# MVPandey/DTS

Measured on AMD Instinct MI355X. Metric: scored_trajectories_per_sec, higher is better.
Workload: dtype bf16

## Files before the change

dts_amd/models/llama.py:

```python

from __future__ import annotations

import math
from typing import Optional

import torch
import torch.nn as nn
import torch.nn.functional as F

from dts_amd import ops
from dts_amd.models.config import ModelSpec
from dts_amd.ops.torch_ref import build_rope_cache
from dts_amd.parallel.tp import (
    ColumnParallelLinear,
    RowParallelLinear,
    TPContext,
    _init_weight,
)
from dts_amd.serving.batch import ForwardBatch


class LlamaAttention(nn.Module):
    def __init__(self, spec: ModelSpec, tp: TPContext, dtype):
        super().__init__()
        self.tp = tp
        assert spec.num_heads % tp.size == 0
        assert spec.num_kv_heads % tp.size == 0 or tp.size % spec.num_kv_heads == 0
        self.num_heads = spec.num_heads // tp.size
        self.num_kv_heads = max(1, spec.num_kv_heads // tp.size)
        self.head_dim = spec.head_dim
        self.scale = 1.0 / math.sqrt(spec.head_dim)
        q_out = self.num_heads * self.head_dim * tp.size
        kv_out = self.num_kv_heads * self.head_dim * tp.size
        self.qkv_proj = ColumnParallelLinear(
            spec.hidden_size, q_out + 2 * kv_out, tp, dtype=dtype
        )
        self.o_proj = RowParallelLinear(
            self.num_heads * self.head_dim * tp.size, spec.hidden_size, tp, dtype=dtype
        )
        self.q_size = self.num_heads * self.head_dim
        self.kv_size = self.num_kv_heads * self.head_dim

    def forward(
        self,
        hidden: torch.Tensor,
        batch: ForwardBatch,
        kv_layer: tuple,
        rope: tuple,
    ) -> torch.Tensor:
        T = hidden.shape[0]
        qkv = self.qkv_proj(hidden)
        q, k, v = qkv.split([self.q_size, self.kv_size, self.kv_size], dim=-1)
        q = q.view(T, self.num_heads, self.head_dim)
        k = k.view(T, self.num_kv_heads, self.head_dim)
        v = v.view(T, self.num_kv_heads, self.head_dim)

        k_cache, v_cache = kv_layer
        cos, sin = rope
        q, k = ops.rope_kv_append(
            q, k, v, batch.positions, cos, sin, k_cache, v_cache, batch.slot_mapping
        )

        out = torch.empty(q.shape, dtype=q.dtype, device=q.device)
        np_tok = batch.num_prefill_tokens
        if batch.num_prefill_seqs:
            ops.attn_prefill_paged(
                q[:np_tok],
                batch.cu_q,
                batch.positions[:np_tok],
                k_cache,
                v_cache,
                batch.prefill_block_tables,
                batch.prefill_kv_lens,
                self.scale,
                out=out[:np_tok],
            )
        if batch.num_decode_seqs:
            ops.attn_decode_paged(
                q[np_tok:],
                k_cache,
                v_cache,
                batch.decode_block_tables,
                batch.decode_kv_lens,
                self.scale,
                out=out[np_tok:],
            )
        return self.o_proj(out.reshape(T, -1))


class LlamaMLP(nn.Module):
    def __init__(self, spec: ModelSpec, tp: TPContext, dtype):
        super().__init__()
        self.gate_up_proj = ColumnParallelLinear(
            spec.hidden_size, 2 * spec.intermediate_size, tp, dtype=dtype
        )
        self.down_proj = RowParallelLinear(
            spec.intermediate_size, spec.hidden_size, tp, dtype=dtype
        )
        self.inter_per_rank = spec.intermediate_size // tp.size

    def forward(self, x: torch.Tensor) -> torch.Tensor:
        gu = self.gate_up_proj(x)
        return self.down_proj(ops.silu_mul(gu))


class LlamaLayer(nn.Module):
    def __init__(self, spec: ModelSpec, tp: TPContext, dtype):
        super().__init__()
        self.input_norm_w = nn.Parameter(
            torch.ones(spec.hidden_size, dtype=dtype), requires_grad=False
        )
        self.post_norm_w = nn.Parameter(
            torch.ones(spec.hidden_size, dtype=dtype), requires_grad=False
        )
        self.attn = LlamaAttention(spec, tp, dtype)
        self.mlp = LlamaMLP(spec, tp, dtype)
        self.eps = spec.rms_eps

    def forward(self, hidden, residual, batch, kv_layer, rope):
        if residual is None:
            residual = hidden
            hidden = ops.rmsnorm(hidden, self.input_norm_w, self.eps)
        else:
            hidden, residual = ops.fused_add_rmsnorm(
                hidden, residual, self.input_norm_w, self.eps
            )
        hidden = self.attn(hidden, batch, kv_layer, rope)
        hidden, residual = ops.fused_add_rmsnorm(
            hidden, residual, self.post_norm_w, self.eps
        )
        hidden = self.mlp(hidden)
        return hidden, residual


class LlamaModel(nn.Module):
    arch = "llama"

    def __init__(
        self,
        spec: ModelSpec,
        tp: Optional[TPContext] = None,
        dtype: torch.dtype = torch.bfloat16,
        device: str = "cpu",
    ):
        super().__init__()
        tp = tp or TPContext.single()
        self.spec = spec
        self.tp = tp
        self.dtype = dtype
        self.num_kv_heads_local = max(1, spec.num_kv_heads // tp.size)
        self.embed = nn.Parameter(
            torch.empty(spec.vocab_size, spec.hidden_size, dtype=dtype),
            requires_grad=False,
        )
        self.layers = nn.ModuleList(
            [LlamaLayer(spec, tp, dtype) for _ in range(spec.num_layers)]
        )
        self.final_norm_w = nn.Parameter(
            torch.ones(spec.hidden_size, dtype=dtype), requires_grad=False
        )
        self.lm_head = ColumnParallelLinear(
            spec.hidden_size, spec.vocab_size, tp, dtype=dtype, gather_output=True
        )
        cos, sin = build_rope_cache(
            spec.head_dim, spec.max_position, spec.rope_theta, dtype=torch.float32
        )
        self.register_buffer("rope_cos", cos, persistent=False)
        self.register_buffer("rope_sin", sin, persistent=False)
        self.to(device)

    def random_init(self, seed: int = 0) -> None:
        dev = self.embed.device
        g = torch.Generator(device=dev).manual_seed(seed)
        spec = self.spec
        with torch.no_grad():
            self.embed.copy_(
                torch.randn(
                    spec.vocab_size, spec.hidden_size, generator=g, device=dev
                )
                .mul_(0.02)
                .to(self.dtype)
            )
            for layer in self.layers:
                for lin in (
                    layer.attn.qkv_proj,
                    layer.attn.o_proj,
                    layer.mlp.gate_up_proj,
                    layer.mlp.down_proj,
                ):
                    lin.weight.copy_(
                        _init_weight(
                            *lin.weight.shape,
                            dtype=self.dtype,
                            generator=g,
                            device=dev,
                        )
                    )
            self.lm_head.weight.copy_(
                _init_weight(
                    *self.lm_head.weight.shape,
                    dtype=self.dtype,
                    generator=g,
                    device=dev,
                )
            )

    def forward(self, batch: ForwardBatch, kv_pool) -> torch.Tensor:
        hidden = self.embed[batch.token_ids]
        residual = None
        rope = (self.rope_cos, self.rope_sin)
        for i, layer in enumerate(self.layers):
            hidden, residual = layer(hidden, residual, batch, kv_pool.layer(i), rope)
        hidden, _ = ops.fused_add_rmsnorm(
            hidden, residual, self.final_norm_w, self.spec.rms_eps
        )
        if batch.sample_indices is not None:
            hidden = hidden[batch.sample_indices]
        return self.lm_head(hidden).float()
```

dts_amd/ops/__init__.py:

```python

from __future__ import annotations

import os

import torch

from dts_amd.ops import torch_ref
from dts_amd.utils.logging import logger

_hip = None
_hip_load_error: Exception | None = None


def _try_load_hip():
    global _hip, _hip_load_error
    if _hip is not None or _hip_load_error is not None:
        return _hip
    try:
        from dts_amd.ops import _hip_ext_loader

        _hip = _hip_ext_loader.load()
        logger.info("HIP extension loaded: %s", _hip.__name__)
    except Exception as e:
        _hip_load_error = e
    return _hip


def hip_available() -> bool:
    return _try_load_hip() is not None


def _require_hip():
    ext = _try_load_hip()
    if ext is None:
        if os.environ.get("DTS_ALLOW_TORCH_FALLBACK") == "1":
            return None
        raise RuntimeError(
            "dts_amd HIP extension not available on a GPU device "
            f"(load error: {_hip_load_error}); refusing silent eager fallback. "
            "Build with `python -m dts_amd.ops.build` or set "
            "DTS_ALLOW_TORCH_FALLBACK=1 for debugging."
        )
    return ext


def _on_gpu(t: torch.Tensor) -> bool:
    return t.is_cuda



def rmsnorm(x, weight, eps=1e-5):
    if _on_gpu(x):
        ext = _require_hip()
        if ext is not None:
            out = torch.empty_like(x)
            ext.rmsnorm(out, x, weight, eps)
            return out
    return torch_ref.rmsnorm(x, weight, eps)


def fused_add_rmsnorm(x, residual, weight, eps=1e-5):
    if _on_gpu(x):
        ext = _require_hip()
        if ext is not None:
            ext.fused_add_rmsnorm(x, residual, weight, eps)
            return x, residual
    return torch_ref.fused_add_rmsnorm(x, residual, weight, eps)


def layernorm(x, weight, bias, eps=1e-5):
    if _on_gpu(x):
        ext = _require_hip()
        if ext is not None:
            out = torch.empty_like(x)
            ext.layernorm(out, x, weight, bias, eps)
            return out
    return torch_ref.layernorm(x, weight, bias, eps)


def rope_kv_append(q, k, v, positions, cos, sin, k_cache, v_cache, slot_mapping):
    if _on_gpu(q):
        ext = _require_hip()
        if ext is not None:
            ext.rope_kv_append(q, k, v, positions, cos, sin, k_cache, v_cache, slot_mapping)
            return q, k
    q, k = torch_ref.rope_apply(q, k, positions, cos, sin)
    torch_ref.kv_append(k, v, k_cache, v_cache, slot_mapping)
    return q, k


def kv_append(k, v, k_cache, v_cache, slot_mapping):
    if _on_gpu(k):
        ext = _require_hip()
        if ext is not None:
            ext.kv_append(k, v, k_cache, v_cache, slot_mapping)
            return
    torch_ref.kv_append(k, v, k_cache, v_cache, slot_mapping)


def attn_prefill_paged(
    q, cu_q, q_positions, k_cache, v_cache, block_tables, kv_lens, scale=None,
    out=None,
):
    if _on_gpu(q):
        ext = _require_hip()
        if ext is not None:
            import math

            if out is None or not out.is_contiguous():
                out = torch.empty(q.shape, dtype=q.dtype, device=q.device)
            ext.attn_prefill_paged(
                out, q, cu_q, q_positions, k_cache, v_cache, block_tables, kv_lens,
                scale if scale is not None else 1.0 / math.sqrt(q.shape[-1]),
            )
            return out
    ref = torch_ref.attn_prefill_paged(
        q, cu_q, q_positions, k_cache, v_cache, block_tables, kv_lens, scale
    )
    if out is not None:
        out.copy_(ref)
        return out
    return ref


def attn_decode_paged(q, k_cache, v_cache, block_tables, kv_lens, scale=None, out=None):
    if _on_gpu(q):
        ext = _require_hip()
        if ext is not None:
            import math

            if out is None or not out.is_contiguous():
                out = torch.empty(q.shape, dtype=q.dtype, device=q.device)
            ext.attn_decode_paged(
                out, q, k_cache, v_cache, block_tables, kv_lens,
                scale if scale is not None else 1.0 / math.sqrt(q.shape[-1]),
            )
            return out
    ref = torch_ref.attn_decode_paged(q, k_cache, v_cache, block_tables, kv_lens, scale)
    if out is not None:
        out.copy_(ref)
        return out
    return ref


def silu_mul(gate_up):
    if gate_up.shape[0] == 0:
        return gate_up[:, : gate_up.shape[1] // 2]
    if _on_gpu(gate_up):
        ext = _require_hip()
        if ext is not None:
            T = gate_up.shape[0]
            out = torch.empty(
                (T, gate_up.shape[1] // 2), dtype=gate_up.dtype, device=gate_up.device
            )
            ext.silu_mul(out, gate_up)
            return out
    return torch_ref.silu_mul(gate_up)


def gelu(x):
    return torch_ref.gelu(x)


_sampler_ws: dict = {}


def _sampler_workspace(S: int, device):
    key = (str(device), S)
    ws = _sampler_ws.get(key)
    if ws is None:
        ws = (
            torch.zeros(S, dtype=torch.int64, device=device),
            torch.zeros(S, 1024, dtype=torch.float32, device=device),
            torch.zeros(S, 16, dtype=torch.float32, device=device),
            torch.zeros(S, dtype=torch.float32, device=device),
        )
        _sampler_ws[key] = ws
    return ws


def top_p_sample(logits, temperatures, top_ps, generators=None, seeds=None, out=None):
    if _on_gpu(logits):
        ext = _require_hip()
        if ext is not None and seeds is not None:
            S, V = logits.shape
            if out is None:
                out = torch.empty(S, dtype=torch.long, device=logits.device)
            if V >= 4096 and S <= 32 and os.environ.get("DTS_SAMPLER_V1") != "1":
                ws = _sampler_workspace(S, logits.device)
                ext.top_p_sample_v2(
                    out, logits, temperatures, top_ps, seeds, *ws
                )
            else:
                ext.top_p_sample(out, logits, temperatures, top_ps, seeds)
            return out
    return torch_ref.top_p_sample(logits, temperatures, top_ps, generators)


def derive_seeds(out, bases, positions):
    if _on_gpu(out):
        ext = _require_hip()
        if ext is not None:
            ext.derive_seeds(out, bases, positions)
            return out
    out.copy_(torch_ref.derive_seeds(bases, positions))
    return out


mix_seed = torch_ref.mix_seed


def moe_grouped_linear(x, w, counts, offsets):
    if _on_gpu(x):
        ext = _require_hip()
        if ext is not None:
            out = torch.empty(
                (x.shape[0], w.shape[1]), dtype=x.dtype, device=x.device
            )
            ext.moe_grouped_linear(out, x, w, counts, offsets)
            return out
    return torch_ref.moe_grouped_linear(x, w, counts, offsets)


def linear_bf16(x: torch.Tensor, weight: torch.Tensor) -> torch.Tensor:
    M = x.shape[0] if x.dim() == 2 else 0
    if (
        x.is_cuda
        and x.dtype == torch.bfloat16
        and x.dim() == 2
        and x.shape[1] % 512 == 0
        and weight.stride(1) == 1
        and 1 <= M <= 16
    ):
        ext = _require_hip()
        if ext is not None:
            out = torch.empty(
                (M, weight.shape[0]), dtype=x.dtype, device=x.device
            )
            big = weight.shape[0] * weight.shape[1] * 2 > (96 << 20)
            if M <= 2 and big and x.shape[1] <= 8192:
                ext.gemv_bf16(out, x, weight)
            else:
                ext.gemm_skinny_bf16(out, x, weight)
            return out
    return torch.nn.functional.linear(x, weight)
```

dts_amd/ops/hip/bindings.cpp:

```cpp
#include <torch/extension.h>

void rmsnorm(torch::Tensor out, torch::Tensor x, torch::Tensor w, double eps);
void fused_add_rmsnorm(torch::Tensor x, torch::Tensor residual,
                       torch::Tensor w, double eps);
void silu_mul(torch::Tensor out, torch::Tensor in);
void layernorm(torch::Tensor out, torch::Tensor x, torch::Tensor w,
               torch::Tensor b, double eps);
void rope_kv_append(torch::Tensor q, torch::Tensor k, torch::Tensor v,
                    torch::Tensor positions, torch::Tensor cos_t,
                    torch::Tensor sin_t, torch::Tensor k_cache,
                    torch::Tensor v_cache, torch::Tensor slots);
void kv_append(torch::Tensor k, torch::Tensor v, torch::Tensor k_cache,
               torch::Tensor v_cache, torch::Tensor slots);
void attn_decode_paged(torch::Tensor out, torch::Tensor q,
                       torch::Tensor kcache, torch::Tensor vcache,
                       torch::Tensor block_tables, torch::Tensor kv_lens,
                       double scale);
void attn_prefill_paged(torch::Tensor out, torch::Tensor q, torch::Tensor cu_q,
                        torch::Tensor q_pos, torch::Tensor kcache,
                        torch::Tensor vcache, torch::Tensor block_tables,
                        torch::Tensor kv_lens, double scale, int64_t swz);
void top_p_sample(torch::Tensor out, torch::Tensor logits, torch::Tensor temps,
                  torch::Tensor top_ps, torch::Tensor seeds);
void derive_seeds(torch::Tensor out, torch::Tensor bases,
                  torch::Tensor positions);
void top_p_sample_v2(torch::Tensor out, torch::Tensor logits,
                     torch::Tensor temps, torch::Tensor top_ps,
                     torch::Tensor seeds, torch::Tensor ws_max,
                     torch::Tensor ws_bins, torch::Tensor ws_slice,
                     torch::Tensor ws_tau);
void gemv_bf16(torch::Tensor out, torch::Tensor x, torch::Tensor w);
void gemm_skinny_bf16(torch::Tensor out, torch::Tensor x, torch::Tensor w);
void moe_grouped_linear(torch::Tensor out, torch::Tensor x, torch::Tensor w,
                        torch::Tensor counts, torch::Tensor offsets);

PYBIND11_MODULE(TORCH_EXTENSION_NAME, m) {
  m.def("rmsnorm", &rmsnorm, "RMSNorm (bf16, CDNA4)");
  m.def("fused_add_rmsnorm", &fused_add_rmsnorm,
        "fused residual add + RMSNorm (in-place, bf16)");
  m.def("silu_mul", &silu_mul, "SwiGLU activation (bf16)");
  m.def("layernorm", &layernorm, "LayerNorm (bf16, GPT-2 path)");
  m.def("rope_kv_append", &rope_kv_append,
        "fused rotate-half RoPE + paged KV append (bf16)");
  m.def("kv_append", &kv_append, "paged KV append without RoPE (bf16)");
  m.def("attn_decode_paged", &attn_decode_paged,
        "paged GQA decode attention (bf16, wave-per-kv-head)");
  m.def("attn_prefill_paged", &attn_prefill_paged,
        "paged causal prefill attention (bf16, MFMA)", py::arg("out"),
        py::arg("q"), py::arg("cu_q"), py::arg("q_pos"), py::arg("kcache"),
        py::arg("vcache"), py::arg("block_tables"), py::arg("kv_lens"),
        py::arg("scale"), py::arg("swz") = -1);
  m.def("top_p_sample", &top_p_sample,
        "fused temperature softmax + top-p sampling (sort-free)");
  m.def("derive_seeds", &derive_seeds,
        "stateless (seed, position) mix for chained decode");
  m.def("top_p_sample_v2", &top_p_sample_v2,
        "gridded top-p sampler (vocab sliced across workgroups)");
  m.def("gemv_bf16", &gemv_bf16,
        "skinny-batch (M<=8) bf16 weight-streaming GEMV");
  m.def("gemm_skinny_bf16", &gemm_skinny_bf16,
        "skinny-M (M<=16) bf16 MFMA weight-streaming GEMM");
  m.def("moe_grouped_linear", &moe_grouped_linear,
        "grouped per-expert skinny GEMM (capture-safe MoE decode)");
}
```

dts_amd/ops/hip/common.h:

```cpp
#pragma once

#include <hip/hip_runtime.h>
#include <hip/hip_bf16.h>
#include <hip/hip_fp16.h>

#define WAVE 64
#define DEV __device__ __forceinline__

typedef __attribute__((ext_vector_type(4))) short short4v;
typedef __attribute__((ext_vector_type(8))) short short8v;
typedef __attribute__((ext_vector_type(4))) float float4v;

DEV float bf2f(short u) {
  union { float f; unsigned int i; } c;
  c.i = ((unsigned int)(unsigned short)u) << 16;
  return c.f;
}

DEV short f2bf(float f) {
  union { float f; unsigned int i; } c;
  c.f = f;
  unsigned int lsb = (c.i >> 16) & 1;
  c.i += 0x7fff + lsb;
  return (short)(c.i >> 16);
}

DEV float wave_sum(float v) {
#pragma unroll
  for (int off = 32; off > 0; off >>= 1) v += __shfl_xor(v, off, 64);
  return v;
}

DEV float wave_max(float v) {
#pragma unroll
  for (int off = 32; off > 0; off >>= 1) v = fmaxf(v, __shfl_xor(v, off, 64));
  return v;
}

#define HIP_CHECK_LAST()                                                      \
  do {                                                                        \
    hipError_t e = hipGetLastError();                                         \
    if (e != hipSuccess) {                                                    \
      TORCH_CHECK(false, "HIP kernel launch failed: ", hipGetErrorString(e)); \
    }                                                                         \
  } while (0)
```

dts_amd/ops/hip/elementwise.hip:

```cpp

#include "common.h"
#include <torch/extension.h>
#include <c10/hip/HIPStream.h>


template <int BLOCK>
__global__ void rmsnorm_kernel(short* __restrict__ out,
                               const short* __restrict__ x,
                               const short* __restrict__ w, float eps, int T,
                               int H) {
  __shared__ float red[BLOCK / WAVE];
  for (int row = blockIdx.x; row < T; row += gridDim.x) {
    const short* xr = x + (long)row * H;
    short* yr = out + (long)row * H;
    float ss = 0.f;
    for (int i = threadIdx.x * 8; i < H; i += BLOCK * 8) {
      short8v v = *(const short8v*)(xr + i);
#pragma unroll
      for (int j = 0; j < 8; ++j) {
        float f = bf2f(v[j]);
        ss += f * f;
      }
    }
    ss = wave_sum(ss);
    if ((threadIdx.x & (WAVE - 1)) == 0) red[threadIdx.x / WAVE] = ss;
    __syncthreads();
    float tot = 0.f;
#pragma unroll
    for (int i = 0; i < BLOCK / WAVE; ++i) tot += red[i];
    float inv = rsqrtf(tot / H + eps);
    for (int i = threadIdx.x * 8; i < H; i += BLOCK * 8) {
      short8v v = *(const short8v*)(xr + i);
      short8v wv = *(const short8v*)(w + i);
      short8v o;
#pragma unroll
      for (int j = 0; j < 8; ++j) o[j] = f2bf(bf2f(v[j]) * inv * bf2f(wv[j]));
      *(short8v*)(yr + i) = o;
    }
    __syncthreads();
  }
}


template <int BLOCK>
__global__ void fused_add_rmsnorm_kernel(short* __restrict__ x,
                                         short* __restrict__ residual,
                                         const short* __restrict__ w,
                                         float eps, int T, int H) {
  __shared__ float red[BLOCK / WAVE];
  for (int row = blockIdx.x; row < T; row += gridDim.x) {
    short* xr = x + (long)row * H;
    short* rr = residual + (long)row * H;
    float ss = 0.f;
    for (int i = threadIdx.x * 8; i < H; i += BLOCK * 8) {
      short8v xv = *(const short8v*)(xr + i);
      short8v rv = *(const short8v*)(rr + i);
      short8v nv;
#pragma unroll
      for (int j = 0; j < 8; ++j) {
        float s = bf2f(xv[j]) + bf2f(rv[j]);
        nv[j] = f2bf(s);
        float f = bf2f(nv[j]);
        ss += f * f;
      }
      *(short8v*)(rr + i) = nv;
    }
    ss = wave_sum(ss);
    if ((threadIdx.x & (WAVE - 1)) == 0) red[threadIdx.x / WAVE] = ss;
    __syncthreads();
    float tot = 0.f;
#pragma unroll
    for (int i = 0; i < BLOCK / WAVE; ++i) tot += red[i];
    float inv = rsqrtf(tot / H + eps);
    for (int i = threadIdx.x * 8; i < H; i += BLOCK * 8) {
      short8v rv = *(const short8v*)(rr + i);
      short8v wv = *(const short8v*)(w + i);
      short8v o;
#pragma unroll
      for (int j = 0; j < 8; ++j) o[j] = f2bf(bf2f(rv[j]) * inv * bf2f(wv[j]));
      *(short8v*)(xr + i) = o;
    }
    __syncthreads();
  }
}


template <int BLOCK>
__global__ void layernorm_kernel(short* __restrict__ out,
                                 const short* __restrict__ x,
                                 const short* __restrict__ w,
                                 const short* __restrict__ b, float eps,
                                 int T, int H) {
  __shared__ float red[BLOCK / WAVE];
  for (int row = blockIdx.x; row < T; row += gridDim.x) {
    const short* xr = x + (long)row * H;
    short* yr = out + (long)row * H;
    float sum = 0.f;
    for (int i = threadIdx.x * 8; i < H; i += BLOCK * 8) {
      short8v v = *(const short8v*)(xr + i);
#pragma unroll
      for (int j = 0; j < 8; ++j) sum += bf2f(v[j]);
    }
    sum = wave_sum(sum);
    if ((threadIdx.x & (WAVE - 1)) == 0) red[threadIdx.x / WAVE] = sum;
    __syncthreads();
    float tot = 0.f;
#pragma unroll
    for (int i = 0; i < BLOCK / WAVE; ++i) tot += red[i];
    const float mu = tot / H;
    __syncthreads();
    float ss = 0.f;
    for (int i = threadIdx.x * 8; i < H; i += BLOCK * 8) {
      short8v v = *(const short8v*)(xr + i);
#pragma unroll
      for (int j = 0; j < 8; ++j) {
        float d = bf2f(v[j]) - mu;
        ss += d * d;
      }
    }
    ss = wave_sum(ss);
    if ((threadIdx.x & (WAVE - 1)) == 0) red[threadIdx.x / WAVE] = ss;
    __syncthreads();
    float vtot = 0.f;
#pragma unroll
    for (int i = 0; i < BLOCK / WAVE; ++i) vtot += red[i];
    const float inv = rsqrtf(vtot / H + eps);
    for (int i = threadIdx.x * 8; i < H; i += BLOCK * 8) {
      short8v v = *(const short8v*)(xr + i);
      short8v wv = *(const short8v*)(w + i);
      short8v bv = *(const short8v*)(b + i);
      short8v o;
#pragma unroll
      for (int j = 0; j < 8; ++j)
        o[j] = f2bf((bf2f(v[j]) - mu) * inv * bf2f(wv[j]) + bf2f(bv[j]));
      *(short8v*)(yr + i) = o;
    }
    __syncthreads();
  }
}


__global__ void silu_mul_kernel(short* __restrict__ out,
                                const short* __restrict__ in, long T, long I) {
  long idx = ((long)blockIdx.x * blockDim.x + threadIdx.x) * 8;
  long total = T * I;
  for (; idx < total; idx += (long)gridDim.x * blockDim.x * 8) {
    long t = idx / I, i = idx % I;
    short8v g = *(const short8v*)(in + t * 2 * I + i);
    short8v u = *(const short8v*)(in + t * 2 * I + I + i);
    short8v o;
#pragma unroll
    for (int j = 0; j < 8; ++j) {
      float gf = bf2f(g[j]);
      float s = gf / (1.f + __expf(-gf));
      o[j] = f2bf(s * bf2f(u[j]));
    }
    *(short8v*)(out + t * I + i) = o;
  }
}


__global__ void rope_kv_append_kernel(
    short* __restrict__ q, short* __restrict__ k, const short* __restrict__ v,
    const long* __restrict__ positions, const float* __restrict__ cos_t,
    const float* __restrict__ sin_t, short* __restrict__ k_cache,
    short* __restrict__ v_cache, const long* __restrict__ slots, int T, int Hq,
    int Hk, int D, int BS, long cache_head_stride, long cache_block_stride,
    int do_rope, long q_tstride, long k_tstride, long v_tstride) {
  int unit = blockIdx.x * (blockDim.x / WAVE) + threadIdx.x / WAVE;
  int lane = threadIdx.x & (WAVE - 1);
  int units = T * (Hq + 2 * Hk);
  if (unit >= units) return;
  int t = unit / (Hq + 2 * Hk);
  int h = unit % (Hq + 2 * Hk);
  long pos = positions[t];
  int half = D / 2;

  if (do_rope && h < Hq + Hk) {
    short* base = (h < Hq) ? q + (long)t * q_tstride + (long)h * D
                           : k + (long)t * k_tstride + (long)(h - Hq) * D;
    for (int i = lane; i < half; i += WAVE) {
      float c = cos_t[pos * half + i];
      float s = sin_t[pos * half + i];
      float x1 = bf2f(base[i]);
      float x2 = bf2f(base[i + half]);
      base[i] = f2bf(x1 * c - x2 * s);
      base[i + half] = f2bf(x2 * c + x1 * s);
    }
  }
  if (h >= Hq) {
    bool is_v = h >= Hq + Hk;
    int kvh = is_v ? (h - Hq - Hk) : (h - Hq);
    const short* src = is_v ? v + (long)t * v_tstride + (long)kvh * D
                            : k + (long)t * k_tstride + (long)kvh * D;
    short* cache = is_v ? v_cache : k_cache;
    long slot = slots[t];
    long block = slot / BS, off = slot % BS;
    short* dst = cache + block * cache_block_stride + kvh * cache_head_stride +
                 off * D;
    for (int i = lane * 2; i < D; i += WAVE * 2) {
      *(int*)(dst + i) = *(const int*)(src + i);
    }
  }
}


static inline int grid_rows(int T) { return T < 2048 ? T : 2048; }

void rmsnorm(torch::Tensor out, torch::Tensor x, torch::Tensor w, double eps) {
  TORCH_CHECK(x.scalar_type() == torch::kBFloat16 && x.is_contiguous());
  int T = x.numel() / x.size(-1), H = x.size(-1);
  TORCH_CHECK(H % (256 * 8) == 0 || H % 8 == 0, "H must be multiple of 8");
  hipLaunchKernelGGL((rmsnorm_kernel<256>), dim3(grid_rows(T)), dim3(256), 0,
                     c10::hip::getCurrentHIPStream(),
                     (short*)out.data_ptr(), (const short*)x.data_ptr(),
                     (const short*)w.data_ptr(), (float)eps, T, H);
  HIP_CHECK_LAST();
}

void fused_add_rmsnorm(torch::Tensor x, torch::Tensor residual,
                       torch::Tensor w, double eps) {
  TORCH_CHECK(x.scalar_type() == torch::kBFloat16 && x.is_contiguous());
  int T = x.numel() / x.size(-1), H = x.size(-1);
  hipLaunchKernelGGL((fused_add_rmsnorm_kernel<256>), dim3(grid_rows(T)),
                     dim3(256), 0, c10::hip::getCurrentHIPStream(),
                     (short*)x.data_ptr(), (short*)residual.data_ptr(),
                     (const short*)w.data_ptr(), (float)eps, T, H);
  HIP_CHECK_LAST();
}

void layernorm(torch::Tensor out, torch::Tensor x, torch::Tensor w,
               torch::Tensor b, double eps) {
  TORCH_CHECK(x.scalar_type() == torch::kBFloat16 && x.is_contiguous());
  int T = x.numel() / x.size(-1), H = x.size(-1);
  TORCH_CHECK(H % 8 == 0);
  hipLaunchKernelGGL((layernorm_kernel<256>), dim3(grid_rows(T)), dim3(256),
                     0, c10::hip::getCurrentHIPStream(),
                     (short*)out.data_ptr(), (const short*)x.data_ptr(),
                     (const short*)w.data_ptr(), (const short*)b.data_ptr(),
                     (float)eps, T, H);
  HIP_CHECK_LAST();
}

void silu_mul(torch::Tensor out, torch::Tensor in) {
  TORCH_CHECK(in.scalar_type() == torch::kBFloat16 && in.is_contiguous());
  long T = in.size(0), I = in.size(1) / 2;
  TORCH_CHECK(I % 8 == 0);
  long total = T * I / 8;
  int blocks = (int)std::min<long>((total + 255) / 256, 2048);
  hipLaunchKernelGGL(silu_mul_kernel, dim3(blocks), dim3(256), 0,
                     c10::hip::getCurrentHIPStream(), (short*)out.data_ptr(),
                     (const short*)in.data_ptr(), T, I);
  HIP_CHECK_LAST();
}

static inline void check_qkv_layout(const torch::Tensor& t) {
  TORCH_CHECK(t.dim() == 3 && t.stride(2) == 1 && t.stride(1) == t.size(2),
              "expected [T,H,D] with dense heads; got strides ", t.strides());
}

void rope_kv_append(torch::Tensor q, torch::Tensor k, torch::Tensor v,
                    torch::Tensor positions, torch::Tensor cos_t,
                    torch::Tensor sin_t, torch::Tensor k_cache,
                    torch::Tensor v_cache, torch::Tensor slots) {
  TORCH_CHECK(q.scalar_type() == torch::kBFloat16);
  TORCH_CHECK(cos_t.scalar_type() == torch::kFloat32);
  check_qkv_layout(q);
  check_qkv_layout(k);
  check_qkv_layout(v);
  int T = q.size(0), Hq = q.size(1), D = q.size(2), Hk = k.size(1);
  int BS = k_cache.size(2);
  long head_stride = k_cache.stride(1), block_stride = k_cache.stride(0);
  int units = T * (Hq + 2 * Hk);
  int waves_per_block = 4;
  int blocks = (units + waves_per_block - 1) / waves_per_block;
  hipLaunchKernelGGL(rope_kv_append_kernel, dim3(blocks),
                     dim3(waves_per_block * WAVE), 0,
                     c10::hip::getCurrentHIPStream(), (short*)q.data_ptr(),
                     (short*)k.data_ptr(), (const short*)v.data_ptr(),
                     (const long*)positions.data_ptr(),
                     (const float*)cos_t.data_ptr(),
                     (const float*)sin_t.data_ptr(),
                     (short*)k_cache.data_ptr(), (short*)v_cache.data_ptr(),
                     (const long*)slots.data_ptr(), T, Hq, Hk, D, BS,
                     head_stride, block_stride, 1, q.stride(0), k.stride(0),
                     v.stride(0));
  HIP_CHECK_LAST();
}

void kv_append(torch::Tensor k, torch::Tensor v, torch::Tensor k_cache,
               torch::Tensor v_cache, torch::Tensor slots) {
  int T = k.size(0), Hk = k.size(1), D = k.size(2);
  int BS = k_cache.size(2);
  long head_stride = k_cache.stride(1), block_stride = k_cache.stride(0);
  int units = T * (0 + 2 * Hk);
  int blocks = (units + 3) / 4;
  hipLaunchKernelGGL(rope_kv_append_kernel, dim3(blocks), dim3(256), 0,
                     c10::hip::getCurrentHIPStream(), (short*)k.data_ptr(),
                     (short*)k.data_ptr(), (const short*)v.data_ptr(),
                     (const long*)slots.data_ptr(), nullptr, nullptr,
                     (short*)k_cache.data_ptr(), (short*)v_cache.data_ptr(),
                     (const long*)slots.data_ptr(), T, 0, Hk, D, BS,
                     head_stride, block_stride, 0, 0, k.stride(0),
                     v.stride(0));
  HIP_CHECK_LAST();
}
```

dts_amd/ops/hip/gemm_skinny.hip:

```cpp

#include "common.h"
#include <torch/extension.h>
#include <c10/hip/HIPStream.h>

using bf16x8 = __attribute__((ext_vector_type(8))) short;
using f32x4 = __attribute__((ext_vector_type(4))) float;

#define NWAVES 4
#define KSTEP 32
#define KUNROLL 4

template <int KU>
__global__ void __launch_bounds__(NWAVES* WAVE)
gemm_skinny_kernel(short* __restrict__ out,
                   const short* __restrict__ x,
                   const short* __restrict__ w,
                   int M, int N, int K, long x_ts, long out_ts) {
  const int wave = threadIdx.x / WAVE;
  const int lane = threadIdx.x & (WAVE - 1);
  const int n0 = blockIdx.x * 16;

  const int kq = K / NWAVES;
  const int kbeg = wave * kq;
  const int kend = kbeg + kq;

  const int a_row = lane & 15;
  const int k_off = (lane >> 4) * 8;
  const int b_row = n0 + (lane & 15);
  const bool a_live = a_row < M;
  const bool b_live = b_row < N;
  const short* xrow = x + (long)a_row * x_ts;
  const short* wrow = w + (long)b_row * K;

  f32x4 acc = {0.f, 0.f, 0.f, 0.f};
  const bf16x8 zero8 = {0, 0, 0, 0, 0, 0, 0, 0};

  for (int k0 = kbeg; k0 < kend; k0 += KSTEP * KU) {
    bf16x8 a[KU], b[KU];
#pragma unroll
    for (int u = 0; u < KU; ++u) {
      const int kk = k0 + u * KSTEP + k_off;
      a[u] = a_live ? *(const bf16x8*)(xrow + kk) : zero8;
      b[u] = b_live ? *(const bf16x8*)(wrow + kk) : zero8;
    }
#pragma unroll
    for (int u = 0; u < KU; ++u)
      acc = __builtin_amdgcn_mfma_f32_16x16x32_bf16(a[u], b[u], acc, 0, 0, 0);
  }

  __shared__ float red[NWAVES][16][16];
  const int c_col = lane & 15;
#pragma unroll
  for (int i = 0; i < 4; ++i) red[wave][(lane >> 4) * 4 + i][c_col] = acc[i];
  __syncthreads();
  if (wave == 0) {
#pragma unroll
    for (int i = 0; i < 4; ++i) {
      const int m = (lane >> 4) * 4 + i;
      const int n = n0 + c_col;
      if (m < M && n < N) {
        float v = red[0][m][c_col] + red[1][m][c_col] + red[2][m][c_col] +
                  red[3][m][c_col];
        out[(long)m * out_ts + n] = f2bf(v);
      }
    }
  }
}


__global__ void __launch_bounds__(NWAVES* WAVE)
moe_grouped_kernel(short* __restrict__ out,
                   const short* __restrict__ x,
                   const short* __restrict__ w,
                   const int* __restrict__ counts,
                   const int* __restrict__ offsets,
                   int N, int K) {
  const int wave = threadIdx.x / WAVE;
  const int lane = threadIdx.x & (WAVE - 1);
  const int n0 = blockIdx.x * 16;
  const int e = blockIdx.y;
  const int cnt = counts[e];
  if (cnt == 0) return;
  const int off = offsets[e];
  const short* we = w + (long)e * N * K;

  const int kq = K / NWAVES;
  const int kbeg = wave * kq;
  const int kend = kbeg + kq;
  const int a_row = lane & 15;
  const int k_off = (lane >> 4) * 8;
  const int b_row = n0 + (lane & 15);
  const bool b_live = b_row < N;
  const short* wrow = we + (long)b_row * K;
  const bf16x8 zero8 = {0, 0, 0, 0, 0, 0, 0, 0};

  __shared__ float red[NWAVES][16][16];
  const int c_col = lane & 15;

  for (int mb = 0; mb < cnt; mb += 16) {
    const bool a_live = mb + a_row < cnt;
    const short* xrow = x + (long)(off + mb + a_row) * K;
    f32x4 acc = {0.f, 0.f, 0.f, 0.f};
    for (int k0 = kbeg; k0 < kend; k0 += KSTEP * KUNROLL) {
      bf16x8 a[KUNROLL], b[KUNROLL];
#pragma unroll
      for (int u = 0; u < KUNROLL; ++u) {
        const int kk = k0 + u * KSTEP + k_off;
        a[u] = a_live ? *(const bf16x8*)(xrow + kk) : zero8;
        b[u] = b_live ? *(const bf16x8*)(wrow + kk) : zero8;
      }
#pragma unroll
      for (int u = 0; u < KUNROLL; ++u)
        acc = __builtin_amdgcn_mfma_f32_16x16x32_bf16(a[u], b[u], acc, 0, 0, 0);
    }
#pragma unroll
    for (int i = 0; i < 4; ++i) red[wave][(lane >> 4) * 4 + i][c_col] = acc[i];
    __syncthreads();
    if (wave == 0) {
#pragma unroll
      for (int i = 0; i < 4; ++i) {
        const int m = (lane >> 4) * 4 + i;
        const int n = n0 + c_col;
        if (mb + m < cnt && n < N) {
          float v = red[0][m][c_col] + red[1][m][c_col] + red[2][m][c_col] +
                    red[3][m][c_col];
          out[(long)(off + mb + m) * N + n] = f2bf(v);
        }
      }
    }
    __syncthreads();
  }
}

void moe_grouped_linear(torch::Tensor out, torch::Tensor x, torch::Tensor w,
                        torch::Tensor counts, torch::Tensor offsets) {
  TORCH_CHECK(x.scalar_type() == torch::kBFloat16 && x.is_contiguous());
  TORCH_CHECK(w.is_contiguous(), "expert weights must be contiguous [E,N,K]");
  TORCH_CHECK(out.is_contiguous());
  TORCH_CHECK(counts.scalar_type() == torch::kInt32 &&
              offsets.scalar_type() == torch::kInt32);
  const int K = x.size(1), E = w.size(0), N = w.size(1);
  TORCH_CHECK(K % (NWAVES * KSTEP * KUNROLL) == 0, "K must be /512");
  const int tiles = (N + 15) / 16;
  hipLaunchKernelGGL(moe_grouped_kernel, dim3(tiles, E), dim3(NWAVES * WAVE),
                     0, c10::hip::getCurrentHIPStream(),
                     (short*)out.data_ptr(), (const short*)x.data_ptr(),
                     (const short*)w.data_ptr(),
                     (const int*)counts.data_ptr(),
                     (const int*)offsets.data_ptr(), N, K);
  HIP_CHECK_LAST();
}

void gemm_skinny_bf16(torch::Tensor out, torch::Tensor x, torch::Tensor w) {
  TORCH_CHECK(x.scalar_type() == torch::kBFloat16);
  TORCH_CHECK(w.is_contiguous(), "weight must be contiguous [N, K]");
  TORCH_CHECK(x.stride(1) == 1, "x rows must be dense");
  TORCH_CHECK(out.stride(1) == 1);
  const int M = x.size(0), K = x.size(1), N = w.size(0);
  TORCH_CHECK(M >= 1 && M <= 16, "skinny path is for M<=16");
  TORCH_CHECK(K % (NWAVES * KSTEP * KUNROLL) == 0, "K must be /512");
  const int tiles = (N + 15) / 16;
  static const int ku = [] {
    const char* e = getenv("DTS_SKINNY_UNROLL");
    return (e && e[0] == '8') ? 8 : 4;
  }();
  auto stream = c10::hip::getCurrentHIPStream();
  if (ku == 8 && K % (NWAVES * KSTEP * 8) == 0)
    hipLaunchKernelGGL((gemm_skinny_kernel<8>), dim3(tiles),
                       dim3(NWAVES * WAVE), 0, stream, (short*)out.data_ptr(),
                       (const short*)x.data_ptr(), (const short*)w.data_ptr(),
                       M, N, K, x.stride(0), out.stride(0));
  else
    hipLaunchKernelGGL((gemm_skinny_kernel<4>), dim3(tiles),
                       dim3(NWAVES * WAVE), 0, stream, (short*)out.data_ptr(),
                       (const short*)x.data_ptr(), (const short*)w.data_ptr(),
                       M, N, K, x.stride(0), out.stride(0));
  HIP_CHECK_LAST();
}
```

Baseline: 0.3727.

## Fuse SwiGLU into skinny gate_up GEMM and add multi-tile workgroups

Adds a gemm_skinny_swiglu path in which each workgroup computes one gate tile and its matching up tile and applies SiLU-multiply in the epilogue. This removes the separate silu_mul kernel and the round trip of the [M,2I] intermediate for decode-sized batches (M between 8 and 16). The skinny GEMM also becomes templated on the number of N-tiles per workgroup, with an automatic choice by M and tile count, and unroll now defaults to 8 when K >= 8192. These change grid sizes and register pressure, which can cost occupancy, and the gate and up values are rounded to bf16 before the SiLU.

```diff
diff --git a/dts_amd/models/llama.py b/dts_amd/models/llama.py
--- a/dts_amd/models/llama.py
+++ b/dts_amd/models/llama.py
@@ -100,8 +100,9 @@
         self.inter_per_rank = spec.intermediate_size // tp.size
 
     def forward(self, x: torch.Tensor) -> torch.Tensor:
-        gu = self.gate_up_proj(x)
-        return self.down_proj(ops.silu_mul(gu))
+        gup = self.gate_up_proj
+        assert gup.bias is None and not gup.gather_output
+        return self.down_proj(ops.linear_swiglu(x, gup.weight))
 
 
 class LlamaLayer(nn.Module):
diff --git a/dts_amd/ops/__init__.py b/dts_amd/ops/__init__.py
--- a/dts_amd/ops/__init__.py
+++ b/dts_amd/ops/__init__.py
@@ -223,8 +223,24 @@
 
 
 def linear_bf16(x: torch.Tensor, weight: torch.Tensor) -> torch.Tensor:
+    kind = _skinny_kind(x, weight)
+    if kind is not None:
+        ext = _require_hip()
+        if ext is not None:
+            out = torch.empty(
+                (x.shape[0], weight.shape[0]), dtype=x.dtype, device=x.device
+            )
+            if kind == "gemv":
+                ext.gemv_bf16(out, x, weight)
+            else:
+                ext.gemm_skinny_bf16(out, x, weight)
+            return out
+    return torch.nn.functional.linear(x, weight)
+
+
+def _skinny_kind(x: torch.Tensor, weight: torch.Tensor) -> str | None:
     M = x.shape[0] if x.dim() == 2 else 0
-    if (
+    if not (
         x.is_cuda
         and x.dtype == torch.bfloat16
         and x.dim() == 2
@@ -232,15 +248,24 @@
         and weight.stride(1) == 1
         and 1 <= M <= 16
     ):
-        ext = _require_hip()
-        if ext is not None:
-            out = torch.empty(
-                (M, weight.shape[0]), dtype=x.dtype, device=x.device
-            )
-            big = weight.shape[0] * weight.shape[1] * 2 > (96 << 20)
-            if M <= 2 and big and x.shape[1] <= 8192:
-                ext.gemv_bf16(out, x, weight)
-            else:
-                ext.gemm_skinny_bf16(out, x, weight)
-            return out
-    return torch.nn.functional.linear(x, weight)
+        return None
+    big = weight.shape[0] * weight.shape[1] * 2 > (96 << 20)
+    if M <= 2 and big and x.shape[1] <= 8192:
+        return "gemv"
+    return "skinny"
+
+
+def linear_swiglu(x: torch.Tensor, weight: torch.Tensor) -> torch.Tensor:
+    if (
+        _skinny_kind(x, weight) == "skinny"
+        and x.shape[0] >= 8
+        and weight.shape[0] % 32 == 0
+    ):
+        ext = _require_hip()
+        if ext is not None:
+            out = torch.empty(
+                (x.shape[0], weight.shape[0] // 2), dtype=x.dtype, device=x.device
+            )
+            ext.gemm_skinny_swiglu_bf16(out, x, weight)
+            return out
+    return silu_mul(linear_bf16(x, weight))
diff --git a/dts_amd/ops/hip/bindings.cpp b/dts_amd/ops/hip/bindings.cpp
--- a/dts_amd/ops/hip/bindings.cpp
+++ b/dts_amd/ops/hip/bindings.cpp
@@ -30,7 +30,10 @@
                      torch::Tensor ws_bins, torch::Tensor ws_slice,
                      torch::Tensor ws_tau);
 void gemv_bf16(torch::Tensor out, torch::Tensor x, torch::Tensor w);
-void gemm_skinny_bf16(torch::Tensor out, torch::Tensor x, torch::Tensor w);
+void gemm_skinny_bf16(torch::Tensor out, torch::Tensor x, torch::Tensor w,
+                      int64_t tiles_per_wg, int64_t unroll);
+void gemm_skinny_swiglu_bf16(torch::Tensor out, torch::Tensor x,
+                             torch::Tensor w);
 void moe_grouped_linear(torch::Tensor out, torch::Tensor x, torch::Tensor w,
                         torch::Tensor counts, torch::Tensor offsets);
 
@@ -59,7 +62,14 @@
   m.def("gemv_bf16", &gemv_bf16,
         "skinny-batch (M<=8) bf16 weight-streaming GEMV");
   m.def("gemm_skinny_bf16", &gemm_skinny_bf16,
-        "skinny-M (M<=16) bf16 MFMA weight-streaming GEMM");
+        "skinny-M (M<=16) bf16 MFMA weight-streaming GEMM; tiles_per_wg "
+        "pins the N-tiles per workgroup (1/2/4), unroll the k-chunks in "
+        "flight (4/8; 8 needs K % 1024 == 0); 0 = auto",
+        py::arg("out"), py::arg("x"), py::arg("w"),
+        py::arg("tiles_per_wg") = 0, py::arg("unroll") = 0);
+  m.def("gemm_skinny_swiglu_bf16", &gemm_skinny_swiglu_bf16,
+        "skinny-M gate_up GEMM with fused SwiGLU epilogue: "
+        "out[M,I] = silu(x Wg^T) * (x Wu^T), w = [Wg; Wu]");
   m.def("moe_grouped_linear", &moe_grouped_linear,
         "grouped per-expert skinny GEMM (capture-safe MoE decode)");
 }
diff --git a/dts_amd/ops/hip/common.h b/dts_amd/ops/hip/common.h
--- a/dts_amd/ops/hip/common.h
+++ b/dts_amd/ops/hip/common.h
@@ -25,6 +25,12 @@
   return (short)(c.i >> 16);
 }
 
+DEV short swiglu_bf16(short gate, short up) {
+  float gf = bf2f(gate);
+  float s = gf / (1.f + __expf(-gf));
+  return f2bf(s * bf2f(up));
+}
+
 DEV float wave_sum(float v) {
 #pragma unroll
   for (int off = 32; off > 0; off >>= 1) v += __shfl_xor(v, off, 64);
diff --git a/dts_amd/ops/hip/elementwise.hip b/dts_amd/ops/hip/elementwise.hip
--- a/dts_amd/ops/hip/elementwise.hip
+++ b/dts_amd/ops/hip/elementwise.hip
@@ -150,11 +150,7 @@
     short8v u = *(const short8v*)(in + t * 2 * I + I + i);
     short8v o;
 #pragma unroll
-    for (int j = 0; j < 8; ++j) {
-      float gf = bf2f(g[j]);
-      float s = gf / (1.f + __expf(-gf));
-      o[j] = f2bf(s * bf2f(u[j]));
-    }
+    for (int j = 0; j < 8; ++j) o[j] = swiglu_bf16(g[j], u[j]);
     *(short8v*)(out + t * I + i) = o;
   }
 }
diff --git a/dts_amd/ops/hip/gemm_skinny.hip b/dts_amd/ops/hip/gemm_skinny.hip
--- a/dts_amd/ops/hip/gemm_skinny.hip
+++ b/dts_amd/ops/hip/gemm_skinny.hip
@@ -10,15 +10,17 @@
 #define KSTEP 32
 #define KUNROLL 4
 
-template <int KU>
+template <int KU, int NT, bool SWIGLU>
 __global__ void __launch_bounds__(NWAVES* WAVE)
 gemm_skinny_kernel(short* __restrict__ out,
                    const short* __restrict__ x,
                    const short* __restrict__ w,
-                   int M, int N, int K, long x_ts, long out_ts) {
+                   int M, int N, int K, long x_ts, long out_ts,
+                   int wg_stride, int tile_stride) {
+  static_assert(!SWIGLU || NT == 2, "SwiGLU pairs one gate and one up tile");
   const int wave = threadIdx.x / WAVE;
   const int lane = threadIdx.x & (WAVE - 1);
-  const int n0 = blockIdx.x * 16;
+  const int n0 = blockIdx.x * wg_stride;
 
   const int kq = K / NWAVES;
   const int kbeg = wave * kq;
@@ -26,42 +28,80 @@
 
   const int a_row = lane & 15;
   const int k_off = (lane >> 4) * 8;
-  const int b_row = n0 + (lane & 15);
   const bool a_live = a_row < M;
-  const bool b_live = b_row < N;
   const short* xrow = x + (long)a_row * x_ts;
-  const short* wrow = w + (long)b_row * K;
-
-  f32x4 acc = {0.f, 0.f, 0.f, 0.f};
+  bool b_live[NT];
+  const short* wrow[NT];
+#pragma unroll
+  for (int j = 0; j < NT; ++j) {
+    const int b_row = n0 + j * tile_stride + (lane & 15);
+    b_live[j] = b_row < N;
+    wrow[j] = w + (long)(b_live[j] ? b_row : 0) * K;
+  }
+
+  f32x4 acc[NT];
+#pragma unroll
+  for (int j = 0; j < NT; ++j) acc[j] = {0.f, 0.f, 0.f, 0.f};
   const bf16x8 zero8 = {0, 0, 0, 0, 0, 0, 0, 0};
 
-  for (int k0 = kbeg; k0 < kend; k0 += KSTEP * KU) {
-    bf16x8 a[KU], b[KU];
+  auto load_group = [&](int k0, bf16x8 (&a)[KU], bf16x8 (&b)[NT][KU]) {
 #pragma unroll
     for (int u = 0; u < KU; ++u) {
       const int kk = k0 + u * KSTEP + k_off;
       a[u] = a_live ? *(const bf16x8*)(xrow + kk) : zero8;
-      b[u] = b_live ? *(const bf16x8*)(wrow + kk) : zero8;
-    }
+#pragma unroll
+      for (int j = 0; j < NT; ++j)
+        b[j][u] = b_live[j] ? *(const bf16x8*)(wrow[j] + kk) : zero8;
+    }
+  };
+  auto mfma_group = [&](const bf16x8 (&a)[KU], const bf16x8 (&b)[NT][KU]) {
 #pragma unroll
     for (int u = 0; u < KU; ++u)
-      acc = __builtin_amdgcn_mfma_f32_16x16x32_bf16(a[u], b[u], acc, 0, 0, 0);
-  }
-
-  __shared__ float red[NWAVES][16][16];
+#pragma unroll
+      for (int j = 0; j < NT; ++j)
+        acc[j] = __builtin_amdgcn_mfma_f32_16x16x32_bf16(a[u], b[j][u], acc[j],
+                                                         0, 0, 0);
+  };
+  for (int k0 = kbeg; k0 < kend; k0 += KSTEP * KU) {
+    bf16x8 a[KU], b[NT][KU];
+    load_group(k0, a, b);
+    mfma_group(a, b);
+  }
+
+  __shared__ float red[NT][NWAVES][16][16];
   const int c_col = lane & 15;
 #pragma unroll
-  for (int i = 0; i < 4; ++i) red[wave][(lane >> 4) * 4 + i][c_col] = acc[i];
+  for (int j = 0; j < NT; ++j)
+#pragma unroll
+    for (int i = 0; i < 4; ++i)
+      red[j][wave][(lane >> 4) * 4 + i][c_col] = acc[j][i];
   __syncthreads();
-  if (wave == 0) {
-#pragma unroll
-    for (int i = 0; i < 4; ++i) {
-      const int m = (lane >> 4) * 4 + i;
-      const int n = n0 + c_col;
-      if (m < M && n < N) {
-        float v = red[0][m][c_col] + red[1][m][c_col] + red[2][m][c_col] +
-                  red[3][m][c_col];
-        out[(long)m * out_ts + n] = f2bf(v);
+  if constexpr (SWIGLU) {
+    if (wave == 0) {
+#pragma unroll
+      for (int i = 0; i < 4; ++i) {
+        const int m = (lane >> 4) * 4 + i;
+        const int n = n0 + c_col;
+        if (m < M && n < tile_stride) {
+          float g = red[0][0][m][c_col] + red[0][1][m][c_col] +
+                    red[0][2][m][c_col] + red[0][3][m][c_col];
+          float u = red[1][0][m][c_col] + red[1][1][m][c_col] +
+                    red[1][2][m][c_col] + red[1][3][m][c_col];
+          out[(long)m * out_ts + n] = swiglu_bf16(f2bf(g), f2bf(u));
+        }
+      }
+    }
+  } else {
+    for (int j = wave; j < NT; j += NWAVES) {
+#pragma unroll
+      for (int i = 0; i < 4; ++i) {
+        const int m = (lane >> 4) * 4 + i;
+        const int n = n0 + j * tile_stride + c_col;
+        if (m < M && n < N) {
+          float v = red[j][0][m][c_col] + red[j][1][m][c_col] +
+                    red[j][2][m][c_col] + red[j][3][m][c_col];
+          out[(long)m * out_ts + n] = f2bf(v);
+        }
       }
     }
   }
@@ -151,7 +191,34 @@
   HIP_CHECK_LAST();
 }
 
-void gemm_skinny_bf16(torch::Tensor out, torch::Tensor x, torch::Tensor w) {
+static int skinny_unroll(int K, int64_t unroll) {
+  static const int env_ku = [] {
+    const char* e = getenv("DTS_SKINNY_UNROLL");
+    return (e && e[0] == '8') ? 8 : (e && e[0] == '4') ? 4 : 0;
+  }();
+  TORCH_CHECK(unroll != 8 || K % (NWAVES * KSTEP * 8) == 0,
+              "unroll=8 needs K % 1024 == 0, got K=", K);
+  int ku = unroll ? (int)unroll : env_ku ? env_ku : (K >= 8192 ? 8 : 4);
+  if (K % (NWAVES * KSTEP * 8) != 0) ku = 4;
+  return ku;
+}
+
+#define SKINNY_LAUNCH(KU_, NT_, SW_, grid_, wgs_, ts_)                        \
+  hipLaunchKernelGGL((gemm_skinny_kernel<KU_, NT_, SW_>), dim3(grid_),       \
+                     dim3(NWAVES * WAVE), 0, stream, (short*)out.data_ptr(), \
+                     (const short*)x.data_ptr(), (const short*)w.data_ptr(), \
+                     M, N, K, x.stride(0), out.stride(0), wgs_, ts_)
+
+static int skinny_auto_tiles(int M, int tiles) {
+  if (M < 8) return 1;
+  if (tiles >= 4096) return 4;
+  if (tiles >= 1024) return M > 8 ? 4 : 1;
+  if (tiles >= 384) return 2;
+  return 1;
+}
+
+void gemm_skinny_bf16(torch::Tensor out, torch::Tensor x, torch::Tensor w,
+                      int64_t tiles_per_wg, int64_t unroll) {
   TORCH_CHECK(x.scalar_type() == torch::kBFloat16);
   TORCH_CHECK(w.is_contiguous(), "weight must be contiguous [N, K]");
   TORCH_CHECK(x.stride(1) == 1, "x rows must be dense");
@@ -159,21 +226,47 @@
   const int M = x.size(0), K = x.size(1), N = w.size(0);
   TORCH_CHECK(M >= 1 && M <= 16, "skinny path is for M<=16");
   TORCH_CHECK(K % (NWAVES * KSTEP * KUNROLL) == 0, "K must be /512");
+  TORCH_CHECK(w.size(1) == K && out.size(0) == M && out.size(1) == N);
+  TORCH_CHECK(tiles_per_wg == 0 || tiles_per_wg == 1 || tiles_per_wg == 2 ||
+                  tiles_per_wg == 4,
+              "tiles_per_wg must be 0 (auto), 1, 2 or 4");
+  TORCH_CHECK(unroll == 0 || unroll == 4 || unroll == 8,
+              "unroll must be 0 (auto), 4 or 8");
   const int tiles = (N + 15) / 16;
-  static const int ku = [] {
-    const char* e = getenv("DTS_SKINNY_UNROLL");
-    return (e && e[0] == '8') ? 8 : 4;
-  }();
+  const int nt =
+      tiles_per_wg ? (int)tiles_per_wg : skinny_auto_tiles(M, tiles);
+  const int grid = (tiles + nt - 1) / nt;
   auto stream = c10::hip::getCurrentHIPStream();
-  if (ku == 8 && K % (NWAVES * KSTEP * 8) == 0)
-    hipLaunchKernelGGL((gemm_skinny_kernel<8>), dim3(tiles),
-                       dim3(NWAVES * WAVE), 0, stream, (short*)out.data_ptr(),
-                       (const short*)x.data_ptr(), (const short*)w.data_ptr(),
-                       M, N, K, x.stride(0), out.stride(0));
+  if (skinny_unroll(K, unroll) == 8) {
+    if (nt == 4) SKINNY_LAUNCH(8, 4, false, grid, 64, 16);
+    else if (nt == 2) SKINNY_LAUNCH(8, 2, false, grid, 32, 16);
+    else SKINNY_LAUNCH(8, 1, false, grid, 16, 16);
+  } else {
+    if (nt == 4) SKINNY_LAUNCH(4, 4, false, grid, 64, 16);
+    else if (nt == 2) SKINNY_LAUNCH(4, 2, false, grid, 32, 16);
+    else SKINNY_LAUNCH(4, 1, false, grid, 16, 16);
+  }
+  HIP_CHECK_LAST();
+}
+
+void gemm_skinny_swiglu_bf16(torch::Tensor out, torch::Tensor x,
+                             torch::Tensor w) {
+  TORCH_CHECK(x.scalar_type() == torch::kBFloat16);
+  TORCH_CHECK(w.is_contiguous(), "weight must be contiguous [2I, K]");
+  TORCH_CHECK(x.stride(1) == 1, "x rows must be dense");
+  TORCH_CHECK(out.stride(1) == 1);
+  const int M = x.size(0), K = x.size(1), N = w.size(0);
+  const int I = N / 2;
+  TORCH_CHECK(M >= 1 && M <= 16, "skinny path is for M<=16");
+  TORCH_CHECK(K % (NWAVES * KSTEP * KUNROLL) == 0, "K must be /512");
+  TORCH_CHECK(N == 2 * I && I % 16 == 0, "fused SwiGLU needs I % 16 == 0");
+  TORCH_CHECK(w.size(1) == K && out.size(0) == M && out.size(1) == I);
+  const int grid = I / 16;
+  auto stream = c10::hip::getCurrentHIPStream();
+  if (skinny_unroll(K, 0) == 8)
+    SKINNY_LAUNCH(8, 2, true, grid, 16, I);
   else
-    hipLaunchKernelGGL((gemm_skinny_kernel<4>), dim3(tiles),
-                       dim3(NWAVES * WAVE), 0, stream, (short*)out.data_ptr(),
-                       (const short*)x.data_ptr(), (const short*)w.data_ptr(),
-                       M, N, K, x.stride(0), out.stride(0));
+    SKINNY_LAUNCH(4, 2, true, grid, 16, I);
   HIP_CHECK_LAST();
 }
+#undef SKINNY_LAUNCH
```

After: 0.3853, median of 6. 1.03x the previous value.
